# codeandkey/kami

Measured on AMD Instinct MI355X. Metric: NN leaf-evals/sec at batch 512 (119×8×8 planes), 1/2/4/8 MI355X, higher is better.
Workload: dtype bf16

## Files before the change

kami_amd/csrc/kh_api.hip:

```cpp
#include "kh_internal.h"
#include "torch_archive.h"
#include "torch_archive_write.h"

#include <sched.h>
#include <atomic>
#include <chrono>
#include <thread>
#include <cmath>
#include <condition_variable>
#include <cstdarg>
#include <cstdio>
#include <cstdlib>
#include <cstring>
#include <memory>
#include <mutex>
#include <random>
#include <algorithm>
#include <string>
#include <vector>

namespace {

thread_local std::string g_err;

// ... 117 lines not shown
    uint32_t u;
    memcpy(&u, &f, 4);
    if ((u & 0x7fffffffu) > 0x7f800000u) return (uint16_t)((u >> 16) | 0x40);
    u += 0x7fffu + ((u >> 16) & 1u);
    return (uint16_t)(u >> 16);
}
uint16_t f2f16(float f)
{
    _Float16 h = (_Float16)f;
    uint16_t r;
    memcpy(&r, &h, 2);
    return r;
}

void pack_layer(std::vector<uint16_t>& out, int dtype, const float* w, const float* scale, int Co, int Ci,
                int taps, int KS, int MS, int ci0 = 0, bool centre_first = false, int perm = 0, bool pad = true)
{
    int kstep = 0;
    for (int ti = 0; ti < taps; ++ti) {
        const int tap = !centre_first ? ti : (ti == 0 ? 4 : (ti <= 4 ? ti - 1 : ti));
        for (int ks = 0; ks < KS; ++ks, ++kstep)
            for (int ms = 0; ms < MS; ++ms)
                for (int l = 0; l < 64; ++l) {
                    const int r = l & 31, h = l >> 5;
                    for (int j = 0; j < 8; ++j) {
                        const int co = ms * 32 + r;
                        const int ci = ci0 + (kstep < perm ? 32 * (ks >> 1) + 8 * (2 * (ks & 1) + (j >> 2)) + 4 * h + (j & 3)
                                                           : ks * 16 + 8 * h + j);
                        float v = 0.0f;
                        if (co < Co && ci < Ci) v = w[((size_t)co * Ci + ci) * taps + tap] * (scale ? scale[co] : 1.0f);
                        out.push_back(dtype == KH_BF16 ? f2bf16(v) : f2f16(v));
                    }
                }
    }
    while (pad && out.size() % 4096) out.push_back(0);
// ... 154 lines not shown
    return KH_OK;
}

int build_tower(Weights& W, const HostNet& n, int dtype, int F, int C, int R)
{
    using namespace kh;
    if (C > TW_CP) { W.tw_why = "filters > 64 not supported by the MFMA tower kernel yet"; return KH_OK; }
    if (F > 128) { W.tw_why = "features > 128 not supported by the MFMA tower kernel yet"; return KH_OK; }
    const int FP = F <= 32 ? 32 : 128;
    if (tower_lds_bytes(FP, R) > 160 * 1024) { W.tw_why = "too many residual blocks for the LDS parameter area"; return KH_OK; }
    std::vector<float> sc(128), sh(128);
    std::vector<uint16_t> stream;
    std::vector<float> par((size_t)tower_par_copy_floats(R), 0.0f);
    fold_bn(n.stem, C, sc.data(), sh.data());
    if (FP == 128) {
        for (int q = 0; q < 4; ++q) pack_layer(stream, dtype, n.stem.w, sc.data(), C, F, 9, 2, 2, 32 * q, false, 0, false);
        if (stream.size() != (size_t)18 * 4096) return fail(KH_ERR_INVALID, "internal: stem stream size");
    } else {
        pack_layer(stream, dtype, n.stem.w, sc.data(), C, F, 9, FP / 16, 2);
    }
    memcpy(par.data(), sh.data(), sizeof(float) * C);
    for (int i = 0; i < 2 * R; ++i) {
        fold_bn(n.res[i], C, sc.data(), sh.data());
        pack_layer(stream, dtype, n.res[i].w, sc.data(), C, C, 9, TW_CP / 16, 2, 0, true, TW_CP / 16);
        memcpy(par.data() + (size_t)(1 + i) * TW_CP, sh.data(), sizeof(float) * C);
    }
    float* pshift1 = par.data() + (size_t)(1 + 2 * R) * TW_CP;
    fold_bn(n.pconv, KH_POLICY_MID, sc.data(), pshift1);
    pack_layer(stream, dtype, n.pconv.w, sc.data(), KH_POLICY_MID, C, 1, TW_CP / 16, 4, 0, false, TW_CP / 16);
    float* pbias2 = pshift1 + KH_POLICY_MID;
    memcpy(pbias2, n.p2b, sizeof(float) * KH_POLICY_PLANES);
    pack_layer(stream, dtype, n.p2w, nullptr, KH_POLICY_PLANES, KH_POLICY_MID, 1, KH_POLICY_MID / 16, 4, 0, false, KH_POLICY_MID / 16);
    if (((stream.size() / 4096) & 1) != 0) stream.resize(stream.size() + 4096, 0);
    float* vw = pbias2 + 128;
    float vs, vsh;
    fold_bn(n.vconv, 1, &vs, &vsh);
    for (int i = 0; i < C; ++i) vw[i] = n.vconv.w[i] * vs;
    vw[TW_CP] = vsh;
    std::vector<float> fc4((size_t)KH_VALUE_WIDTH * 64 + KH_VALUE_WIDTH);
    for (int j = 0; j < KH_VALUE_WIDTH; ++j)
        for (int k = 0; k < 64; ++k) fc4[((size_t)(k / 4) * KH_VALUE_WIDTH + j) * 4 + (k & 3)] = n.fcw[(size_t)j * 64 + k];
    memcpy(fc4.data() + (size_t)KH_VALUE_WIDTH * 64, n.fcb, sizeof(float) * KH_VALUE_WIDTH);

    W.tw_nchunks = (int)(stream.size() / 4096);
    W.tw_npar = (int)par.size();
    W.tw_FP = FP;
    int rc = 0;
// ... 1775 lines not shown
```

kami_amd/csrc/kh_internal.h:

```cpp
#pragma once
#include <hip/hip_runtime.h>
#include <stddef.h>
#include <stdint.h>

#include "../../include/kami_hip.h"

namespace kh {

void launch_encode_f32(const kh_board* d_boards, int n, float* d_planes, hipStream_t s);

void launch_gather_legal(const float* policy, const int32_t* offsets, const int32_t* actions,
                         float* priors, int B, hipStream_t s, const float* vfull = nullptr, int vstride = 0,
                         float* values = nullptr, const int* flags_in = nullptr, int* flags_out = nullptr);

void launch_signal(unsigned* host_word, unsigned serial, hipStream_t s);

struct SimpleLayer {
    const float* wt;
    const float* scale;
    const float* shift;
    int Ci, Co, taps;
    int relu;
};
void launch_simple_conv(const SimpleLayer& L, const float* in, const float* skip, float* out,
// ... 17 lines not shown
    const float* fcb;
    float* policy;
    float* vfull;
    float* logits;
    int* flags;
    const int32_t* lg_offsets = nullptr;
    const int32_t* lg_actions = nullptr;
    float* lg_priors = nullptr;
    float* lg_values = nullptr;
    int* lg_flags = nullptr;
};

__host__ __device__ constexpr int tower_par_copy_floats(int R) { return (1 + 2 * R) * TW_CP + 128 + 128 + TW_CP + 4; }
__host__ __device__ constexpr int tower_par_floats(int R) { return tower_par_copy_floats(R) + TW_NB * 64 + 16; }
int tower_lds_bytes(int FP, int R);
hipError_t launch_tower(int dtype, int FP, const TowerArgs& a, int num_cus, hipStream_t s);

struct LayersArgs {
    const float* in;
    int B, F, FP, CP, R;
    unsigned short* act_in;
    unsigned short* act[3];
    unsigned short* pmid;
    float* logits;
    float* v64;
    const unsigned short* w;
    const size_t* w_off;
    const unsigned short* w4;
    const size_t* w4_off;
    const float* shift;
// ... 35 lines not shown
```

kami_amd/csrc/tower8_mfma.hip:

```cpp
#include "tower_common.h"

#include <atomic>

namespace kh {

using f32x4_t = float __attribute__((ext_vector_type(4)));
__device__ __forceinline__ void store_wt(f32x4_t* p, f32x4_t v) { asm volatile("global_store_dwordx4 %0, %1, off sc1" ::"v"(p), "v"(v) : "memory"); }
__device__ __forceinline__ void store_wt(float* p, float v) { asm volatile("global_store_dword %0, %1, off sc1" ::"v"(p), "v"(v) : "memory"); }

constexpr int T8_LAG = 1;
struct CPipe { unsigned ring; int cslot; };

__device__ __forceinline__ unsigned cpipe_advance(CPipe& p)
{
    p.cslot = (p.cslot + 1 == RING_D) ? 0 : p.cslot + 1;
    return p.ring + p.cslot * CHUNK;
}

__device__ __forceinline__ unsigned cpipe_step(CPipe& p)
{
    asm volatile("s_barrier" ::: "memory");
    __builtin_amdgcn_sched_barrier(0);
    p.cslot = (p.cslot + 1 == RING_D) ? 0 : p.cslot + 1;
    return p.ring + p.cslot * CHUNK;
// ... 10 lines not shown
                 "global_load_lds_dwordx4 %1, %2 offset:2048\n\tglobal_load_lds_dwordx4 %1, %2 offset:3072\n\t"
                 "s_mov_b32 m0, %0"
                 : "=&s"(keep) : "v"(voff), "s"(sbase), "s"(dst) : "memory");
    p.next = (p.next + 1 == p.nch) ? 0 : p.next + 1;
    p.islot = (p.islot + 1 == RING_D) ? 0 : p.islot + 1;
}

template <int VMX>
__device__ __forceinline__ void hpipe_step(Pipe& p, int hw, int lane)
{
    asm volatile("s_waitcnt vmcnt(%0)" ::"n"(4 * (RING_D - 3 - T8_LAG) + VMX) : "memory");
    asm volatile("s_barrier" ::: "memory");
    pipe_issue4(p, hw, lane);
}

template <typename T, int TAPS, int KS, int MS, int PAR, int NREG = 0, bool CF = false, int TAILV = 0>
__device__ __forceinline__ void gemm8_layer(CPipe& p, const char* smem, int lane, unsigned b_base, int stride,
                                            f32x16 (&acc)[MS], typename Elem<T>::vec8 (&A)[2][8],
                                            const typename Elem<T>::vec8* breg = nullptr)
{
    using V = typename Elem<T>::vec8;
    using S = LayerShape<TAPS, KS, MS>;
    constexpr int KPC = S::KPC;
    V B[2][KPC];
#pragma unroll
    for (int k = 0; k < KPC; ++k) {
        if (k < NREG) B[PAR][k] = breg[k];
        else B[PAR][k] = *reinterpret_cast<const V*>(smem + b_base + b_offset<TAPS, KS, CF>(k, stride));
    }
#pragma unroll
    for (int n = 0; n < S::NCH; ++n) {
        const int cur = (PAR + n) & 1, nxt = cur ^ 1;
        const unsigned a_off = cpipe_step(p) + lane * 16;
#pragma unroll
        for (int f = 0; f < 8; ++f) A[nxt][f] = *reinterpret_cast<const V*>(smem + a_off + f * 1024);
        if (n + 1 < S::NCH) {
#pragma unroll
            for (int k = 0; k < KPC; ++k) {
                if ((n + 1) * KPC + k < NREG) B[nxt][k] = breg[(n + 1) * KPC + k];
                else B[nxt][k] = *reinterpret_cast<const V*>(smem + b_base + b_offset<TAPS, KS, CF>((n + 1) * KPC + k, stride));
            }
        }
        if (TAILV > 0 && n == S::NCH - 1) {
#pragma unroll
            for (int ms = 0; ms < MS; ++ms)
#pragma unroll
                for (int k = 0; k < KPC; ++k) acc[ms] = Elem<T>::mfma(A[cur][k * MS + ms], B[cur][k], acc[ms]);
#pragma unroll
            for (int i = 0; i < KPC; ++i) {
                __builtin_amdgcn_sched_group_barrier(0x100, 2, 0);
                __builtin_amdgcn_sched_group_barrier(0x008, 1, 0);
            }
#pragma unroll
            for (int i = 0; i < (MS - 1) * KPC; ++i) {
                __builtin_amdgcn_sched_group_barrier(0x008, 1, 0);
// ... 11 lines not shown
            __builtin_amdgcn_sched_group_barrier(0x008, 1, 0);
        }
    }
}

template <typename T, int PAR>
__device__ __forceinline__ void gemm8_dummy(CPipe& p, const char* smem, int lane, typename Elem<T>::vec8 (&A)[2][8])
{
    using V = typename Elem<T>::vec8;
    const unsigned a_off = cpipe_step(p) + lane * 16;
#pragma unroll
    for (int f = 0; f < 8; ++f) A[PAR ^ 1][f] = *reinterpret_cast<const V*>(smem + a_off + f * 1024);
}


enum { BM_RASTER = 0, BM_CENTRE = 1, BM_QUARTERS = 2 };
template <int TAPS, int KS, int BM>
__device__ __forceinline__ constexpr unsigned b_off8(int kk, int stride)
{
    if constexpr (BM == BM_QUARTERS) {
        const int pass = kk / (TAPS * KS / 4), k = kk % (TAPS * KS / 4);
        return b_offset<TAPS, KS / 4, false>(k, stride) + pass * (KS / 4) * 32;
    }
    return b_offset<TAPS, KS, BM == BM_CENTRE>(kk, stride);
}

template <typename T, int TAPS, int KS, int MS, int PAR, int NREG, int BM, int N0, int N1, bool BARMID = false>
__device__ __forceinline__ void gemm8_steps(CPipe& p, const char* smem, int lane, unsigned b_base, int stride,
                                            f32x16 (&acc)[MS], typename Elem<T>::vec8 (&A)[2][8],
                                            typename Elem<T>::vec8 (&B)[2][8 / MS],
                                            const typename Elem<T>::vec8* breg = nullptr)
{
    using V = typename Elem<T>::vec8;
    using S = LayerShape<TAPS, KS, MS>;
    constexpr int KPC = S::KPC;
#pragma unroll
    for (int n = N0; n < N1; ++n) {
        const int cur = (PAR + n) & 1, nxt = cur ^ 1;
        if (BARMID && n == N0) {
            static_assert(!BARMID || (MS == 2 && KPC == 4), "mid-step barrier: 2 x 4 chunk");
            const unsigned a_off = cpipe_advance(p) + lane * 16;
#pragma unroll
            for (int k = 0; k < 2; ++k) {
#pragma unroll
                for (int ms = 0; ms < 2; ++ms) {
                    const int i = 2 * k + ms;
                    A[nxt][2 * i] = *reinterpret_cast<const V*>(smem + a_off + (2 * i) * 1024);
                    A[nxt][2 * i + 1] = *reinterpret_cast<const V*>(smem + a_off + (2 * i + 1) * 1024);
                    acc[ms] = Elem<T>::mfma(A[cur][k * MS + ms], B[cur][k], acc[ms]);
                    __builtin_amdgcn_sched_barrier(0);
                }
            }
            asm volatile("s_barrier" ::: "memory");
#pragma unroll
            for (int k = 2; k < 4; ++k) {
#pragma unroll
                for (int ms = 0; ms < 2; ++ms) {
                    if (k == 2 && n + 1 < S::NCH) {
#pragma unroll
                        for (int j = 0; j < 2; ++j) {
                            const int kk = 2 * ms + j;
                            if ((n + 1) * KPC + kk < NREG) B[nxt][kk] = breg[(n + 1) * KPC + kk];
                            else B[nxt][kk] = *reinterpret_cast<const V*>(smem + b_base + b_off8<TAPS, KS, BM>((n + 1) * KPC + kk, stride));
                        }
                    }
                    acc[ms] = Elem<T>::mfma(A[cur][k * MS + ms], B[cur][k], acc[ms]);
                    __builtin_amdgcn_sched_barrier(0);
                }
            }
            continue;
        }
        const unsigned a_off = cpipe_step(p) + lane * 16;
#pragma unroll
        for (int f = 0; f < 8; ++f) A[nxt][f] = *reinterpret_cast<const V*>(smem + a_off + f * 1024);
        if (n + 1 < S::NCH) {
#pragma unroll
            for (int k = 0; k < KPC; ++k) {
                if ((n + 1) * KPC + k < NREG) B[nxt][k] = breg[(n + 1) * KPC + k];
                else B[nxt][k] = *reinterpret_cast<const V*>(smem + b_base + b_off8<TAPS, KS, BM>((n + 1) * KPC + k, stride));
            }
        }
#pragma unroll
        for (int k = 0; k < KPC; ++k)
#pragma unroll
            for (int ms = 0; ms < MS; ++ms) acc[ms] = Elem<T>::mfma(A[cur][k * MS + ms], B[cur][k], acc[ms]);
#pragma unroll
        for (int i = 0; i < 8; ++i) {
            __builtin_amdgcn_sched_group_barrier(0x100, 2, 0);
            __builtin_amdgcn_sched_group_barrier(0x008, 1, 0);
        }
    }
}

enum { EPI_STEM = 0, EPI_PACK = 1, EPI_RESID = 2 };

template <typename T, int EPI, int G>
__device__ __forceinline__ u32x2 epi_group(const f32x16& acc, f32x16& xf)
{
    u32x2 o;
    if (EPI == EPI_PACK) {
        o.x = relu_pk(pack2<T>(acc[4 * G + 0], acc[4 * G + 1]));
        o.y = relu_pk(pack2<T>(acc[4 * G + 2], acc[4 * G + 3]));
    } else {
// ... 1 lines not shown
        for (int i = 0; i < 4; ++i) {
            const float t = relu_nan(acc[4 * G + i]);
            xf[4 * G + i] = EPI == EPI_RESID ? xf[4 * G + i] + t : t;
        }
        o.x = pack2<T>(xf[4 * G + 0], xf[4 * G + 1]);
        o.y = pack2<T>(xf[4 * G + 2], xf[4 * G + 3]);
    }
    return o;
}

#define T8_FENCE() __builtin_amdgcn_sched_barrier(0)

template <typename T, int EPI, int CURP>
__device__ __forceinline__ void boundary(CPipe& p, char* smem, int lane, f32x16 (&acc)[2], f32x16 (&nacc)[2],
                                         unsigned nshift, typename Elem<T>::vec8 (&A)[2][8],
                                         typename Elem<T>::vec8 (&B)[2][4], f32x16 (&xf)[2], unsigned out_pix, unsigned nb_base)
{
    using V = typename Elem<T>::vec8;
    constexpr int cur = CURP, nxt = CURP ^ 1;
    u32x2 o[2][4];
#define T8_LDN(ms, g) do { const float4 s_ = *reinterpret_cast<const float4*>(smem + nshift + ((ms) * 32 + 8 * (g)) * 4); \
        nacc[ms][4 * (g) + 0] = s_.x; nacc[ms][4 * (g) + 1] = s_.y; nacc[ms][4 * (g) + 2] = s_.z; nacc[ms][4 * (g) + 3] = s_.w; } while (0)
#define T8_ST(t, g) (*reinterpret_cast<u32x2*>(smem + out_pix + ((t) * 32 + 8 * (g)) * 2) = o[t][g])
#define T8_FRAG(ks) __builtin_bit_cast(V, (u32x4){ o[(ks) >> 1][2 * ((ks) & 1)].x, o[(ks) >> 1][2 * ((ks) & 1)].y, \
                                                   o[(ks) >> 1][2 * ((ks) & 1) + 1].x, o[(ks) >> 1][2 * ((ks) & 1) + 1].y })
    const unsigned a_off = cpipe_step(p) + lane * 16;
#define T8_RDA(set, f, off) (A[set][f] = *reinterpret_cast<const V*>(smem + (off) + (f) * 1024))
    T8_LDN(0, 0); T8_LDN(0, 1); acc[0] = Elem<T>::mfma(A[cur][0], B[cur][0], acc[0]); T8_FENCE();
    T8_LDN(0, 2); T8_LDN(0, 3); acc[0] = Elem<T>::mfma(A[cur][2], B[cur][1], acc[0]); T8_FENCE();
    T8_LDN(1, 0); T8_LDN(1, 1); acc[0] = Elem<T>::mfma(A[cur][4], B[cur][2], acc[0]); T8_FENCE();
    T8_LDN(1, 2); T8_LDN(1, 3); acc[0] = Elem<T>::mfma(A[cur][6], B[cur][3], acc[0]); T8_FENCE();
    T8_RDA(nxt, 0, a_off); T8_RDA(nxt, 1, a_off); acc[1] = Elem<T>::mfma(A[cur][1], B[cur][0], acc[1]); T8_FENCE();
    T8_RDA(nxt, 2, a_off); T8_RDA(nxt, 3, a_off); acc[1] = Elem<T>::mfma(A[cur][3], B[cur][1], acc[1]); T8_FENCE();
    T8_RDA(nxt, 4, a_off); T8_RDA(nxt, 5, a_off);
    o[0][0] = epi_group<T, EPI, 0>(acc[0], xf[0]); o[0][1] = epi_group<T, EPI, 1>(acc[0], xf[0]);
    acc[1] = Elem<T>::mfma(A[cur][5], B[cur][2], acc[1]); T8_FENCE();
    T8_RDA(nxt, 6, a_off); T8_RDA(nxt, 7, a_off);
    o[0][2] = epi_group<T, EPI, 2>(acc[0], xf[0]); o[0][3] = epi_group<T, EPI, 3>(acc[0], xf[0]);
    acc[1] = Elem<T>::mfma(A[cur][7], B[cur][3], acc[1]); T8_FENCE();
    const unsigned a2 = cpipe_advance(p) + lane * 16;
    {
        const V f0 = T8_FRAG(0);
        T8_ST(0, 0); T8_ST(0, 1); T8_RDA(cur, 0, a2);
        nacc[0] = Elem<T>::mfma(A[nxt][0], f0, nacc[0]); T8_FENCE();
        T8_ST(0, 2); T8_ST(0, 3); T8_RDA(cur, 1, a2);
        nacc[1] = Elem<T>::mfma(A[nxt][1], f0, nacc[1]); T8_FENCE();
    }
    {
        const V f1 = T8_FRAG(1);
        T8_RDA(cur, 2, a2); T8_RDA(cur, 3, a2);
        nacc[0] = Elem<T>::mfma(A[nxt][2], f1, nacc[0]); T8_FENCE();
        T8_RDA(cur, 4, a2); T8_RDA(cur, 5, a2);
        o[1][0] = epi_group<T, EPI, 0>(acc[1], xf[1]); o[1][1] = epi_group<T, EPI, 1>(acc[1], xf[1]);
        nacc[1] = Elem<T>::mfma(A[nxt][3], f1, nacc[1]); T8_FENCE();
    }
    {
        const V f2 = T8_FRAG(2);
        o[1][2] = epi_group<T, EPI, 2>(acc[1], xf[1]); o[1][3] = epi_group<T, EPI, 3>(acc[1], xf[1]);
        T8_ST(1, 0); T8_ST(1, 1); T8_ST(1, 2); T8_ST(1, 3);
        nacc[0] = Elem<T>::mfma(A[nxt][4], f2, nacc[0]); T8_FENCE();
        T8_RDA(cur, 6, a2); T8_RDA(cur, 7, a2);
        nacc[1] = Elem<T>::mfma(A[nxt][5], f2, nacc[1]); T8_FENCE();
    }
    {
        const V f3 = T8_FRAG(3);
        asm volatile("s_waitcnt lgkmcnt(2)\n\ts_barrier" ::: "memory");
#pragma unroll
        for (int k = 0; k < 4; ++k) B[cur][k] = *reinterpret_cast<const V*>(smem + nb_base + b_offset<9, TW_CP / 16, true>(4 + k, XSTR));
        nacc[0] = Elem<T>::mfma(A[nxt][6], f3, nacc[0]); T8_FENCE();
        nacc[1] = Elem<T>::mfma(A[nxt][7], f3, nacc[1]); T8_FENCE();
    }
#undef T8_LDN
#undef T8_ST
}

template <typename T, int EPI, int CURP>
__device__ __forceinline__ void tower_tail(CPipe& p, const char* smem, int lane, f32x16 (&acc)[2], typename Elem<T>::vec8 (&A)[2][8],
                                           typename Elem<T>::vec8 (&B)[2][4], f32x16 (&xf)[2], Packed<2>& xk)
{
    using V = typename Elem<T>::vec8;
    constexpr int cur = CURP, nxt = CURP ^ 1;
    const unsigned a_off = cpipe_step(p) + lane * 16;
    T8_RDA(nxt, 0, a_off); T8_RDA(nxt, 1, a_off); acc[0] = Elem<T>::mfma(A[cur][0], B[cur][0], acc[0]); T8_FENCE();
    T8_RDA(nxt, 2, a_off); T8_RDA(nxt, 3, a_off); acc[0] = Elem<T>::mfma(A[cur][2], B[cur][1], acc[0]); T8_FENCE();
    T8_RDA(nxt, 4, a_off); T8_RDA(nxt, 5, a_off); acc[0] = Elem<T>::mfma(A[cur][4], B[cur][2], acc[0]); T8_FENCE();
    T8_RDA(nxt, 6, a_off); T8_RDA(nxt, 7, a_off); acc[0] = Elem<T>::mfma(A[cur][6], B[cur][3], acc[0]); T8_FENCE();
    acc[1] = Elem<T>::mfma(A[cur][1], B[cur][0], acc[1]); T8_FENCE();
    acc[1] = Elem<T>::mfma(A[cur][3], B[cur][1], acc[1]); T8_FENCE();
    xk.o[0][0] = epi_group<T, EPI, 0>(acc[0], xf[0]); xk.o[0][1] = epi_group<T, EPI, 1>(acc[0], xf[0]);
    acc[1] = Elem<T>::mfma(A[cur][5], B[cur][2], acc[1]); T8_FENCE();
    xk.o[0][2] = epi_group<T, EPI, 2>(acc[0], xf[0]); xk.o[0][3] = epi_group<T, EPI, 3>(acc[0], xf[0]);
    acc[1] = Elem<T>::mfma(A[cur][7], B[cur][3], acc[1]); T8_FENCE();
    xk.o[1][0] = epi_group<T, EPI, 0>(acc[1], xf[1]); xk.o[1][1] = epi_group<T, EPI, 1>(acc[1], xf[1]);
    xk.o[1][2] = epi_group<T, EPI, 2>(acc[1], xf[1]); xk.o[1][3] = epi_group<T, EPI, 3>(acc[1], xf[1]);
}
#undef T8_RDA

template <int STRIDE>
__device__ __forceinline__ void zero_halo(char* base, int board_bytes, int t)
{
    const u32x4 z = { 0, 0, 0, 0 };
    for (int i = t; i < TW_NB * NPIX; i += 256) {
        const int pp = i % NPIX, yy = pp / PITCH, xx = pp % PITCH;
        if (yy >= 1 && yy <= 8 && xx >= 1 && xx <= 8) continue;
        char* d = base + (i / NPIX) * board_bytes + pp * STRIDE;
#pragma unroll
        for (int k = 0; k < STRIDE / 16; ++k) *reinterpret_cast<u32x4*>(d + k * 16) = z;
    }
}

template <bool LEGAL>
__device__ __forceinline__ void helper_value_fc(const TowerArgs& a, const float* v64, int b0, int j, int lane)
{
    asm volatile("s_barrier" ::: "memory");
    unsigned voff = (unsigned)j * 16u;
    asm volatile("" : "+v"(voff));
    float4 fcw[16];
#pragma unroll
    for (int k = 0; k < 16; ++k)
        fcw[k] = *reinterpret_cast<const float4*>(reinterpret_cast<const char*>(a.fcw4) + (size_t)k * KH_VALUE_WIDTH * 16 + voff);
    const float fcbias = a.fcb[j];
    __builtin_amdgcn_sched_barrier(0);
// ... 64 lines not shown
    if (wave >= 6) {
        const int pt = tid & 127;
        for (int grp = blockIdx.x; grp < ngroups; grp += gridDim.x) {
            const int b0 = grp * TW_NB;
            if (KS_STEM == 8) {
                float4_u pl[4][8];
                const int lc = pt & 7;
                const int nb = min(TW_NB, a.B - b0);
                const char* gbase = reinterpret_cast<const char*>(a.in + (size_t)b0 * 64 * F);
                unsigned voff[8];
#pragma unroll
                for (int j = 0; j < 8; ++j) {
                    const int ip = (pt >> 3) + 16 * j;
                    voff[j] = (unsigned)((min(ip >> 6, nb - 1) * 64 + (ip & 63)) * F) * 4u;
                }
                const unsigned sdst = LDS_ST + ((((pt >> 6) + 1) * PITCH + ((pt >> 3) & 7) + 1) * SSTR) + 8 * lc;
                unsigned badmax = 0u;
                auto request = [&](int q) {
                    const unsigned cc = (unsigned)min(32 * q + 4 * lc, F - 4) * 4u;
#pragma unroll
                    for (int j = 0; j < 8; ++j)
                        pl[q][j] = __builtin_nontemporal_load(reinterpret_cast<const float4_u*>(gbase + voff[j] + cc));
                };
                auto convert = [&](int q, int j) {
                    float x[4] = { pl[q][j].x, pl[q][j].y, pl[q][j].z, pl[q][j].w };
                    if (32 * q + 32 > F) {
                        const int c = 32 * q + 4 * lc;
                        const int sh = c - min(c, F - 4);
                        float y[4];
#pragma unroll
                        for (int k = 0; k < 4; ++k) {
// ... 26 lines not shown
                }
                const bool bad = badmax >= 0x7f800000u;
                if (__any(bad) && lane == 0) raise_flag<LEGAL>(a, 0);
            } else {
                if (a.boards) {
                    const int bb = pt >> 6, p = pt & 63;
                    float v[32];
#pragma unroll
                    for (int k = 0; k < 32; ++k) v[k] = 0.0f;
                    if (b0 + bb < a.B) {
                        float w[KH_NFEATURES];
                        encode_square(a.boards + (b0 + bb), p, w);
#pragma unroll
                        for (int k = 0; k < KH_NFEATURES; ++k) v[k] = w[k];
                    }
                    char* dst = smem + LDS_ST + bb * SBOARD + (((p >> 3) + 1) * PITCH + (p & 7) + 1) * SSTR;
#pragma unroll
                    for (int c = 0; c < 4; ++c) {
                        u32x4 o;
                        o.x = pack2<T>(v[8 * c + 0], v[8 * c + 1]); o.y = pack2<T>(v[8 * c + 2], v[8 * c + 3]);
                        o.z = pack2<T>(v[8 * c + 4], v[8 * c + 5]); o.w = pack2<T>(v[8 * c + 6], v[8 * c + 7]);
                        *reinterpret_cast<u32x4*>(dst + c * 16) = o;
                    }
                } else {
                    constexpr int CH = FP / 8;
                    constexpr int NIT = TW_NB * 64 * CH / 128;
                    float vin[NIT][8];
                    const int c0 = (pt % CH) * 8;
#pragma unroll
                    for (int j = 0; j < NIT; ++j) {
                        const int i = pt + 128 * j;
// ... 12 lines not shown
                    }
                    bool bad = false;
#pragma unroll
                    for (int j = 0; j < NIT; ++j) {
                        const int i = pt + 128 * j;
                        const int bb = i / (64 * CH), p = (i / CH) & 63;
                        u32x4 o;
                        unsigned w[4];
#pragma unroll
                        for (int k = 0; k < 4; ++k) {
                            const float lo = vin[j][2 * k], hi = vin[j][2 * k + 1];
                            bad = bad || !__builtin_isfinite(lo) || !__builtin_isfinite(hi);
                            w[k] = pack2<T>(lo, hi);
                        }
                        o.x = w[0]; o.y = w[1]; o.z = w[2]; o.w = w[3];
                        *reinterpret_cast<u32x4*>(smem + LDS_ST + bb * SBOARD + (((p >> 3) + 1) * PITCH + (p & 7) + 1) * SSTR + (pt % CH) * 16) = o;
                    }
                    if (__any(bad) && lane == 0) raise_flag<LEGAL>(a, 0);
                }
                lds_barrier();
                for (int i = 0; i < NSTEM; ++i) asm volatile("s_barrier" ::: "memory");
            }
            const int nsteps = 2 * R * NLAYER + NPOL;
            for (int i = 0; i < nsteps; ++i) {
                asm volatile("s_barrier" ::: "memory");
                if (i == 0 && R > 0) {
                    for (int z = 0; z < 2; ++z) zero_halo<XSTR>(smem + LDS_ST, XBOARD, pt + 128 * z);
                    asm volatile("s_waitcnt lgkmcnt(0)" ::: "memory");
                }
            }
            helper_value_fc<LEGAL>(a, v64, b0, tid & 255, lane);
// ... 5 lines not shown
        Pipe pipe;
        pipe.stream = a.wstream; pipe.nch = a.nchunks; pipe.next = 0; pipe.islot = 0; pipe.ring = LDS_RING;
#pragma unroll
        for (int i = 0; i < RING_D - 1; ++i) pipe_issue4(pipe, hw, lane);

        for (int grp = blockIdx.x; grp < ngroups; grp += gridDim.x) {
            asm volatile("s_waitcnt vmcnt(%0)\n\ts_barrier" ::"n"(4 * (RING_D - 3)) : "memory");
            for (int i = 0; i < nsteps; ++i) hpipe_step<0>(pipe, hw, lane);
            helper_value_fc<LEGAL>(a, v64, grp * TW_NB, tid & 255, lane);
            asm volatile("s_barrier" ::: "memory");
        }
        asm volatile("s_waitcnt vmcnt(0)" ::: "memory");
    } else {
        const int h = lane >> 5;
        const int wb = cw >> 1;
        const int lp = PIXMAP[lane & 31];
        const int py = 4 * (cw & 1) + (lp >> 3), px = lp & 7;
        const unsigned xin = LDS_X + wb * XBOARD + (py * PITCH + px) * XSTR + h * 16;
        const unsigned tin = LDS_ST + wb * XBOARD + (py * PITCH + px) * XSTR + h * 16;
        const unsigned sin = LDS_ST + wb * SBOARD + (py * PITCH + px) * SSTR + h * 16;
        const unsigned xout = LDS_X + wb * XBOARD + ((py + 1) * PITCH + px + 1) * XSTR;
        const unsigned tout = LDS_ST + wb * XBOARD + ((py + 1) * PITCH + px + 1) * XSTR;
        unsigned xout_h = xout + 8 * h, tout_h = tout + 8 * h, sh0 = LDS_PAR + 16 * h;
        asm volatile("" : "+v"(xout_h), "+v"(tout_h), "+v"(sh0));

        CPipe pipe;
        pipe.ring = LDS_RING; pipe.cslot = 0;
        {
            const float4* src = reinterpret_cast<const float4*>(a.params);
            float4* dst = reinterpret_cast<float4*>(par);
            const int n4 = a.npar >> 2;
            for (int i0 = 0; i0 < n4; i0 += 4 * 256) {
                const float4 v0 = src[min(i0 + ct, n4 - 1)], v1 = src[min(i0 + 256 + ct, n4 - 1)];
                const float4 v2 = src[min(i0 + 512 + ct, n4 - 1)], v3 = src[min(i0 + 768 + ct, n4 - 1)];
                if (i0 + ct < n4) dst[i0 + ct] = v0;
                if (i0 + 256 + ct < n4) dst[i0 + 256 + ct] = v1;
                if (i0 + 512 + ct < n4) dst[i0 + 512 + ct] = v2;
// ... 9 lines not shown
            zero_halo<XSTR>(smem + LDS_X, XBOARD, ct);
            zero_halo<SSTR>(smem + LDS_ST, SBOARD, ct);
            lds_barrier();
            if (first) {
                first = false;
#pragma unroll
                for (int f = 0; f < 8; ++f) A[0][f] = *reinterpret_cast<const V*>(smem + LDS_RING + lane * 16 + f * 1024);
            }

            Packed<2> xk;
            f32x16 xf[2];
#pragma unroll
            for (int i = 0; i < 16; ++i) { xf[0][i] = 0.0f; xf[1][i] = 0.0f; }
            f32x16 accA[2], accB[2];
            V B[2][4];
            acc_init<2>(accA, shift3, h);
            {
                constexpr int BMS = KS_STEM == 8 ? BM_QUARTERS : BM_RASTER;
#pragma unroll
                for (int k = 0; k < 4; ++k) B[0][k] = *reinterpret_cast<const V*>(smem + sin + b_off8<9, KS_STEM, BMS>(k, SSTR));
                gemm8_steps<T, 9, KS_STEM, 2, 0, 0, BMS, 0, NSTEM - 1>(pipe, smem, lane, sin, SSTR, accA, A, B);
            }
            constexpr int CP1 = P1 ^ 1;
            for (int r = 0; r < R; ++r) {
                boundary<T, EPI_RESID, CP1>(pipe, smem, lane, accA, accB, sh0 + (1 + 2 * r) * TW_CP * 4, A, B, xf, xout_h, xin);
                gemm8_steps<T, 9, TW_CP / 16, 2, P1, 4, BM_CENTRE, 1, 8, true>(pipe, smem, lane, xin, XSTR, accB, A, B);
                boundary<T, EPI_PACK, P1>(pipe, smem, lane, accB, accA, sh0 + (2 + 2 * r) * TW_CP * 4, A, B, xf, tout_h, tin);
                gemm8_steps<T, 9, TW_CP / 16, 2, P1 ^ 1, 4, BM_CENTRE, 1, 8, true>(pipe, smem, lane, tin, XSTR, accA, A, B);
            }
            tower_tail<T, EPI_RESID, CP1>(pipe, smem, lane, accA, A, B, xf, xk);

            {
                f32x2 s01 = { 0.0f, 0.0f }, s23 = { 0.0f, 0.0f };
#pragma unroll
                for (int ms = 0; ms < 2; ++ms)
#pragma unroll
                    for (int g = 0; g < 4; ++g) {
                        using f32x4 = float __attribute__((ext_vector_type(4)));
                        const f32x4 w = *reinterpret_cast<const f32x4*>(vw + ms * 32 + 8 * g + 4 * h);
                        const f32x2 x01 = { xf[ms][4 * g + 0], xf[ms][4 * g + 1] }, x23 = { xf[ms][4 * g + 2], xf[ms][4 * g + 3] };
                        s01 = x01 * w.xy + s01;
                        s23 = x23 * w.zw + s23;
                    }
// ... 140 lines not shown
```

kami_amd/csrc/tower_common.h:

```cpp
#pragma once
#include "kh_internal.h"
#include "encode_square.h"

namespace kh {

using bf16x8 = __attribute__((ext_vector_type(8))) __bf16;
using f16x8 = __attribute__((ext_vector_type(8))) _Float16;
using f32x16 = __attribute__((ext_vector_type(16))) float;
using u32x4 = __attribute__((ext_vector_type(4))) unsigned;
using u32x2 = __attribute__((ext_vector_type(2))) unsigned;
using float4_u = float __attribute__((ext_vector_type(4), aligned(4)));

constexpr int PITCH = 12;
constexpr int NPIX = 10 * PITCH;
constexpr int XSTR = TW_CP * 2 + 16;
constexpr int XBOARD = NPIX * XSTR;
constexpr int PSTR = KH_POLICY_MID * 2 + 16;
constexpr int PBOARD = 64 * PSTR;
constexpr int LBOARD = KH_PSIZE * 4;
constexpr int RING_D = 6;
constexpr int CHUNK = 8192;
constexpr int LDS_RING = 0;
constexpr int LDS_X = RING_D * CHUNK;
constexpr int LDS_ST = LDS_X + TW_NB * XBOARD;
constexpr int ST_MIN = TW_NB * LBOARD - TW_NB * XBOARD + TW_NB * PBOARD;

__host__ __device__ constexpr int st_size(int FP)
{
    int s = TW_NB * NPIX * (FP * 2 + 16);
    return s > ST_MIN ? s : ST_MIN;
}

static __device__ __constant__ const unsigned char PIXMAP[32] = {
    0, 1, 2, 3,
    8, 9, 10, 11, 12, 13, 14, 15,
    4, 5, 6, 7,
    24, 25, 26, 27,
    16, 17, 18, 19, 20, 21, 22, 23,
    28, 29, 30, 31
};

template <typename T> struct Elem;
template <> struct Elem<__bf16> {
    using vec8 = bf16x8;
    static __device__ __forceinline__ f32x16 mfma(vec8 a, vec8 b, f32x16 c) { return __builtin_amdgcn_mfma_f32_32x32x16_bf16(a, b, c, 0, 0, 0); }
};
template <> struct Elem<_Float16> {
    using vec8 = f16x8;
    static __device__ __forceinline__ f32x16 mfma(vec8 a, vec8 b, f32x16 c) { return __builtin_amdgcn_mfma_f32_32x32x16_f16(a, b, c, 0, 0, 0); }
};

using f32x2 = float __attribute__((ext_vector_type(2)));
template <typename T> __device__ __forceinline__ unsigned pack2(float lo, float hi)
{
    using T2 = T __attribute__((ext_vector_type(2)));
// ... 16 lines not shown
    int islot;
    unsigned ring;
};

__device__ __forceinline__ void lds_barrier()
{
    asm volatile("s_waitcnt lgkmcnt(0)\n\ts_barrier" ::: "memory");
}

template <int TAPS, int KS, int MS> struct LayerShape {
    static constexpr int KPC = 8 / MS;
    static constexpr int TK = TAPS * KS;
    static constexpr int NCH = (TK + KPC - 1) / KPC;
};

template <int TAPS, int KS, bool CF = false>
__device__ __forceinline__ constexpr unsigned b_offset(int kk, int stride)
{
    const int k = kk < TAPS * KS ? kk : 0;
    const int ti = k / KS, ks = k % KS;
    const int tap = !CF ? ti : (ti == 0 ? 4 : (ti <= 4 ? ti - 1 : ti));
    return (unsigned)((TAPS == 9 ? ((tap / 3) * PITCH + (tap % 3)) * stride : 0) + ks * 32);
}

template <int MS>
__device__ __forceinline__ void acc_init(f32x16 (&acc)[MS], const float* shift, int h)
{
#pragma unroll
    for (int ms = 0; ms < MS; ++ms)
#pragma unroll
        for (int g = 0; g < 4; ++g) {
            const float4 s = *reinterpret_cast<const float4*>(shift + ms * 32 + 8 * g + 4 * h);
            acc[ms][4 * g + 0] = s.x; acc[ms][4 * g + 1] = s.y; acc[ms][4 * g + 2] = s.z; acc[ms][4 * g + 3] = s.w;
        }
}

template <int MS> struct Packed { u32x2 o[MS][4]; };
// ... 56 lines not shown
```

Baseline: 16.10 million.

## Derive horizontal 3x3 conv taps via DPP lane shifts instead of LDS reads

The 3x3 tower convolutions now load only the dx=0 column of each tap row from LDS. The dx=-1 and dx=+1 fragments are built from it with DPP row shifts (0x111/0x101), and lanes at the board edges are masked to zero. Because columns no longer need halo padding, the LDS board pitch drops from 12 to 8 and the pixel permutation table is removed. Weights are reordered to match the new tap order. This cuts LDS read traffic and footprint, at the cost of extra VALU DPP work and tighter scheduling constraints, with correctness depending on the lane-to-pixel mapping matching DPP row-shift semantics.

```diff
diff --git a/kami_amd/csrc/kh_api.hip b/kami_amd/csrc/kh_api.hip
--- a/kami_amd/csrc/kh_api.hip
+++ b/kami_amd/csrc/kh_api.hip
@@ -155,11 +155,11 @@
 }
 
 void pack_layer(std::vector<uint16_t>& out, int dtype, const float* w, const float* scale, int Co, int Ci,
-                int taps, int KS, int MS, int ci0 = 0, bool centre_first = false, int perm = 0, bool pad = true)
+                int taps, int KS, int MS, int ci0 = 0, int perm = 0, bool pad = true)
 {
     int kstep = 0;
     for (int ti = 0; ti < taps; ++ti) {
-        const int tap = !centre_first ? ti : (ti == 0 ? 4 : (ti <= 4 ? ti - 1 : ti));
+        const int tap = taps == 9 ? kh::tower_tap(ti) : ti;
         for (int ks = 0; ks < KS; ++ks, ++kstep)
             for (int ms = 0; ms < MS; ++ms)
                 for (int l = 0; l < 64; ++l) {
@@ -344,7 +344,7 @@
     std::vector<float> par((size_t)tower_par_copy_floats(R), 0.0f);
     fold_bn(n.stem, C, sc.data(), sh.data());
     if (FP == 128) {
-        for (int q = 0; q < 4; ++q) pack_layer(stream, dtype, n.stem.w, sc.data(), C, F, 9, 2, 2, 32 * q, false, 0, false);
+        for (int q = 0; q < 4; ++q) pack_layer(stream, dtype, n.stem.w, sc.data(), C, F, 9, 2, 2, 32 * q, 0, false);
         if (stream.size() != (size_t)18 * 4096) return fail(KH_ERR_INVALID, "internal: stem stream size");
     } else {
         pack_layer(stream, dtype, n.stem.w, sc.data(), C, F, 9, FP / 16, 2);
@@ -352,15 +352,15 @@
     memcpy(par.data(), sh.data(), sizeof(float) * C);
     for (int i = 0; i < 2 * R; ++i) {
         fold_bn(n.res[i], C, sc.data(), sh.data());
-        pack_layer(stream, dtype, n.res[i].w, sc.data(), C, C, 9, TW_CP / 16, 2, 0, true, TW_CP / 16);
+        pack_layer(stream, dtype, n.res[i].w, sc.data(), C, C, 9, TW_CP / 16, 2, 0, 3 * TW_CP / 16);
         memcpy(par.data() + (size_t)(1 + i) * TW_CP, sh.data(), sizeof(float) * C);
     }
     float* pshift1 = par.data() + (size_t)(1 + 2 * R) * TW_CP;
     fold_bn(n.pconv, KH_POLICY_MID, sc.data(), pshift1);
-    pack_layer(stream, dtype, n.pconv.w, sc.data(), KH_POLICY_MID, C, 1, TW_CP / 16, 4, 0, false, TW_CP / 16);
+    pack_layer(stream, dtype, n.pconv.w, sc.data(), KH_POLICY_MID, C, 1, TW_CP / 16, 4, 0, TW_CP / 16);
     float* pbias2 = pshift1 + KH_POLICY_MID;
     memcpy(pbias2, n.p2b, sizeof(float) * KH_POLICY_PLANES);
-    pack_layer(stream, dtype, n.p2w, nullptr, KH_POLICY_PLANES, KH_POLICY_MID, 1, KH_POLICY_MID / 16, 4, 0, false, KH_POLICY_MID / 16);
+    pack_layer(stream, dtype, n.p2w, nullptr, KH_POLICY_PLANES, KH_POLICY_MID, 1, KH_POLICY_MID / 16, 4, 0, KH_POLICY_MID / 16);
     if (((stream.size() / 4096) & 1) != 0) stream.resize(stream.size() + 4096, 0);
     float* vw = pbias2 + 128;
     float vs, vsh;
diff --git a/kami_amd/csrc/kh_internal.h b/kami_amd/csrc/kh_internal.h
--- a/kami_amd/csrc/kh_internal.h
+++ b/kami_amd/csrc/kh_internal.h
@@ -55,6 +55,11 @@
 __host__ __device__ constexpr int tower_par_copy_floats(int R) { return (1 + 2 * R) * TW_CP + 128 + 128 + TW_CP + 4; }
 __host__ __device__ constexpr int tower_par_floats(int R) { return tower_par_copy_floats(R) + TW_NB * 64 + 16; }
 int tower_lds_bytes(int FP, int R);
+__host__ __device__ constexpr int tower_tap(int ti)
+{
+    const int dy = ti / 3 == 0 ? 0 : (ti / 3 == 1 ? -1 : 1), dx = ti % 3 == 0 ? 0 : (ti % 3 == 1 ? -1 : 1);
+    return (dy + 1) * 3 + dx + 1;
+}
 hipError_t launch_tower(int dtype, int FP, const TowerArgs& a, int num_cus, hipStream_t s);
 
 struct LayersArgs {
diff --git a/kami_amd/csrc/tower8_mfma.hip b/kami_amd/csrc/tower8_mfma.hip
--- a/kami_amd/csrc/tower8_mfma.hip
+++ b/kami_amd/csrc/tower8_mfma.hip
@@ -48,11 +48,12 @@
     pipe_issue4(p, hw, lane);
 }
 
-template <typename T, int TAPS, int KS, int MS, int PAR, int NREG = 0, bool CF = false, int TAILV = 0>
+template <typename T, int TAPS, int KS, int MS, int PAR, int NREG = 0, int TAILV = 0>
 __device__ __forceinline__ void gemm8_layer(CPipe& p, const char* smem, int lane, unsigned b_base, int stride,
                                             f32x16 (&acc)[MS], typename Elem<T>::vec8 (&A)[2][8],
                                             const typename Elem<T>::vec8* breg = nullptr)
 {
+    static_assert(TAPS == 1, "3x3 layers run through gemm8_steps / boundary");
     using V = typename Elem<T>::vec8;
     using S = LayerShape<TAPS, KS, MS>;
     constexpr int KPC = S::KPC;
@@ -60,7 +61,7 @@
 #pragma unroll
     for (int k = 0; k < KPC; ++k) {
         if (k < NREG) B[PAR][k] = breg[k];
-        else B[PAR][k] = *reinterpret_cast<const V*>(smem + b_base + b_offset<TAPS, KS, CF>(k, stride));
+        else B[PAR][k] = *reinterpret_cast<const V*>(smem + b_base + b_offset1<KS>(k));
     }
 #pragma unroll
     for (int n = 0; n < S::NCH; ++n) {
@@ -72,7 +73,7 @@
 #pragma unroll
             for (int k = 0; k < KPC; ++k) {
                 if ((n + 1) * KPC + k < NREG) B[nxt][k] = breg[(n + 1) * KPC + k];
-                else B[nxt][k] = *reinterpret_cast<const V*>(smem + b_base + b_offset<TAPS, KS, CF>((n + 1) * KPC + k, stride));
+                else B[nxt][k] = *reinterpret_cast<const V*>(smem + b_base + b_offset1<KS>((n + 1) * KPC + k));
             }
         }
         if (TAILV > 0 && n == S::NCH - 1) {
@@ -114,26 +115,38 @@
 }
 
 
-enum { BM_RASTER = 0, BM_CENTRE = 1, BM_QUARTERS = 2 };
-template <int TAPS, int KS, int BM>
-__device__ __forceinline__ constexpr unsigned b_off8(int kk, int stride)
-{
-    if constexpr (BM == BM_QUARTERS) {
-        const int pass = kk / (TAPS * KS / 4), k = kk % (TAPS * KS / 4);
-        return b_offset<TAPS, KS / 4, false>(k, stride) + pass * (KS / 4) * 32;
-    }
-    return b_offset<TAPS, KS, BM == BM_CENTRE>(kk, stride);
-}
-
-template <typename T, int TAPS, int KS, int MS, int PAR, int NREG, int BM, int N0, int N1, bool BARMID = false>
+template <class W, int KPC, int PAR, typename V>
+__device__ __forceinline__ void b_fetch(int c, int k0, int k1, V (&B)[2][KPC], const char* smem, unsigned b_base, int stride,
+                                        const V* breg, unsigned ml, unsigned mr)
+{
+    const int set = (PAR + c) & 1;
+#pragma unroll
+    for (int k = k0; k < k1; ++k) {
+        const int kk = c * KPC + k, kind = W::kind(kk);
+        if (kind == BSRC_LDS) {
+            B[set][k] = *reinterpret_cast<const V*>(smem + b_base + W::off(kk, stride));
+        } else if (kind == BSRC_REG) {
+            B[set][k] = breg[kk];
+        } else if (kind == BSRC_ZERO) {
+            B[set][k] = V{};
+        } else {
+            const int sk = W::src(kk);
+            const V v = W::kind(sk) == BSRC_REG ? breg[sk] : B[(PAR + sk / KPC) & 1][sk % KPC];
+            if (kind == BSRC_SHR) B[set][k] = dpp_frag<V, 0x111>(v, ml);
+            else B[set][k] = dpp_frag<V, 0x101>(v, mr);
+        }
+    }
+}
+
+template <typename T, class W, int MS, int PAR, int N0, int N1, bool BARMID = false>
 __device__ __forceinline__ void gemm8_steps(CPipe& p, const char* smem, int lane, unsigned b_base, int stride,
                                             f32x16 (&acc)[MS], typename Elem<T>::vec8 (&A)[2][8],
                                             typename Elem<T>::vec8 (&B)[2][8 / MS],
-                                            const typename Elem<T>::vec8* breg = nullptr)
+                                            const typename Elem<T>::vec8* breg, unsigned ml, unsigned mr)
 {
     using V = typename Elem<T>::vec8;
-    using S = LayerShape<TAPS, KS, MS>;
-    constexpr int KPC = S::KPC;
+    constexpr int KPC = 8 / MS;
+    constexpr int NCH = (W::TK + KPC - 1) / KPC;
 #pragma unroll
     for (int n = N0; n < N1; ++n) {
         const int cur = (PAR + n) & 1, nxt = cur ^ 1;
@@ -156,14 +169,7 @@
             for (int k = 2; k < 4; ++k) {
 #pragma unroll
                 for (int ms = 0; ms < 2; ++ms) {
-                    if (k == 2 && n + 1 < S::NCH) {
-#pragma unroll
-                        for (int j = 0; j < 2; ++j) {
-                            const int kk = 2 * ms + j;
-                            if ((n + 1) * KPC + kk < NREG) B[nxt][kk] = breg[(n + 1) * KPC + kk];
-                            else B[nxt][kk] = *reinterpret_cast<const V*>(smem + b_base + b_off8<TAPS, KS, BM>((n + 1) * KPC + kk, stride));
-                        }
-                    }
+                    if (k == 2 && n + 1 < NCH) b_fetch<W, KPC, PAR>(n + 1, 2 * ms, 2 * ms + 2, B, smem, b_base, stride, breg, ml, mr);
                     acc[ms] = Elem<T>::mfma(A[cur][k * MS + ms], B[cur][k], acc[ms]);
                     __builtin_amdgcn_sched_barrier(0);
                 }
@@ -173,13 +179,7 @@
         const unsigned a_off = cpipe_step(p) + lane * 16;
 #pragma unroll
         for (int f = 0; f < 8; ++f) A[nxt][f] = *reinterpret_cast<const V*>(smem + a_off + f * 1024);
-        if (n + 1 < S::NCH) {
-#pragma unroll
-            for (int k = 0; k < KPC; ++k) {
-                if ((n + 1) * KPC + k < NREG) B[nxt][k] = breg[(n + 1) * KPC + k];
-                else B[nxt][k] = *reinterpret_cast<const V*>(smem + b_base + b_off8<TAPS, KS, BM>((n + 1) * KPC + k, stride));
-            }
-        }
+        if (n + 1 < NCH) b_fetch<W, KPC, PAR>(n + 1, 0, KPC, B, smem, b_base, stride, breg, ml, mr);
 #pragma unroll
         for (int k = 0; k < KPC; ++k)
 #pragma unroll
@@ -187,6 +187,7 @@
 #pragma unroll
         for (int i = 0; i < 8; ++i) {
             __builtin_amdgcn_sched_group_barrier(0x100, 2, 0);
+            __builtin_amdgcn_sched_group_barrier(0x002, 2, 0);
             __builtin_amdgcn_sched_group_barrier(0x008, 1, 0);
         }
     }
@@ -218,7 +219,8 @@
 template <typename T, int EPI, int CURP>
 __device__ __forceinline__ void boundary(CPipe& p, char* smem, int lane, f32x16 (&acc)[2], f32x16 (&nacc)[2],
                                          unsigned nshift, typename Elem<T>::vec8 (&A)[2][8],
-                                         typename Elem<T>::vec8 (&B)[2][4], f32x16 (&xf)[2], unsigned out_pix, unsigned nb_base)
+                                         typename Elem<T>::vec8 (&B)[2][4], typename Elem<T>::vec8 (&fc)[4],
+                                         f32x16 (&xf)[2], unsigned out_pix, unsigned ml)
 {
     using V = typename Elem<T>::vec8;
     constexpr int cur = CURP, nxt = CURP ^ 1;
@@ -244,35 +246,37 @@
     acc[1] = Elem<T>::mfma(A[cur][7], B[cur][3], acc[1]); T8_FENCE();
     const unsigned a2 = cpipe_advance(p) + lane * 16;
     {
-        const V f0 = T8_FRAG(0);
+        fc[0] = T8_FRAG(0);
         T8_ST(0, 0); T8_ST(0, 1); T8_RDA(cur, 0, a2);
-        nacc[0] = Elem<T>::mfma(A[nxt][0], f0, nacc[0]); T8_FENCE();
+        nacc[0] = Elem<T>::mfma(A[nxt][0], fc[0], nacc[0]); T8_FENCE();
         T8_ST(0, 2); T8_ST(0, 3); T8_RDA(cur, 1, a2);
-        nacc[1] = Elem<T>::mfma(A[nxt][1], f0, nacc[1]); T8_FENCE();
+        B[cur][0] = dpp_frag<V, 0x111>(fc[0], ml);
+        nacc[1] = Elem<T>::mfma(A[nxt][1], fc[0], nacc[1]); T8_FENCE();
     }
     {
-        const V f1 = T8_FRAG(1);
+        fc[1] = T8_FRAG(1);
         T8_RDA(cur, 2, a2); T8_RDA(cur, 3, a2);
-        nacc[0] = Elem<T>::mfma(A[nxt][2], f1, nacc[0]); T8_FENCE();
+        nacc[0] = Elem<T>::mfma(A[nxt][2], fc[1], nacc[0]); T8_FENCE();
         T8_RDA(cur, 4, a2); T8_RDA(cur, 5, a2);
         o[1][0] = epi_group<T, EPI, 0>(acc[1], xf[1]); o[1][1] = epi_group<T, EPI, 1>(acc[1], xf[1]);
-        nacc[1] = Elem<T>::mfma(A[nxt][3], f1, nacc[1]); T8_FENCE();
+        B[cur][1] = dpp_frag<V, 0x111>(fc[1], ml);
+        nacc[1] = Elem<T>::mfma(A[nxt][3], fc[1], nacc[1]); T8_FENCE();
     }
     {
-        const V f2 = T8_FRAG(2);
+        fc[2] = T8_FRAG(2);
         o[1][2] = epi_group<T, EPI, 2>(acc[1], xf[1]); o[1][3] = epi_group<T, EPI, 3>(acc[1], xf[1]);
         T8_ST(1, 0); T8_ST(1, 1); T8_ST(1, 2); T8_ST(1, 3);
-        nacc[0] = Elem<T>::mfma(A[nxt][4], f2, nacc[0]); T8_FENCE();
+        nacc[0] = Elem<T>::mfma(A[nxt][4], fc[2], nacc[0]); T8_FENCE();
         T8_RDA(cur, 6, a2); T8_RDA(cur, 7, a2);
-        nacc[1] = Elem<T>::mfma(A[nxt][5], f2, nacc[1]); T8_FENCE();
+        B[cur][2] = dpp_frag<V, 0x111>(fc[2], ml);
+        nacc[1] = Elem<T>::mfma(A[nxt][5], fc[2], nacc[1]); T8_FENCE();
     }
     {
-        const V f3 = T8_FRAG(3);
+        fc[3] = T8_FRAG(3);
         asm volatile("s_waitcnt lgkmcnt(2)\n\ts_barrier" ::: "memory");
-#pragma unroll
-        for (int k = 0; k < 4; ++k) B[cur][k] = *reinterpret_cast<const V*>(smem + nb_base + b_offset<9, TW_CP / 16, true>(4 + k, XSTR));
-        nacc[0] = Elem<T>::mfma(A[nxt][6], f3, nacc[0]); T8_FENCE();
-        nacc[1] = Elem<T>::mfma(A[nxt][7], f3, nacc[1]); T8_FENCE();
+        nacc[0] = Elem<T>::mfma(A[nxt][6], fc[3], nacc[0]); T8_FENCE();
+        B[cur][3] = dpp_frag<V, 0x111>(fc[3], ml);
+        nacc[1] = Elem<T>::mfma(A[nxt][7], fc[3], nacc[1]); T8_FENCE();
     }
 #undef T8_LDN
 #undef T8_ST
@@ -303,13 +307,12 @@
 template <int STRIDE>
 __device__ __forceinline__ void zero_halo(char* base, int board_bytes, int t)
 {
+    constexpr int NP = STRIDE / 16;
     const u32x4 z = { 0, 0, 0, 0 };
-    for (int i = t; i < TW_NB * NPIX; i += 256) {
-        const int pp = i % NPIX, yy = pp / PITCH, xx = pp % PITCH;
-        if (yy >= 1 && yy <= 8 && xx >= 1 && xx <= 8) continue;
-        char* d = base + (i / NPIX) * board_bytes + pp * STRIDE;
-#pragma unroll
-        for (int k = 0; k < STRIDE / 16; ++k) *reinterpret_cast<u32x4*>(d + k * 16) = z;
+    for (int i = t; i < TW_NB * 2 * PITCH * NP; i += 256) {
+        const int px = i / NP, hp = px % (2 * PITCH);
+        const int pp = hp < PITCH ? hp : (NPIX - 2 * PITCH) + hp;
+        *reinterpret_cast<u32x4*>(base + (px / (2 * PITCH)) * board_bytes + pp * STRIDE + (i % NP) * 16) = z;
     }
 }
 
@@ -404,7 +407,7 @@
                     const int ip = (pt >> 3) + 16 * j;
                     voff[j] = (unsigned)((min(ip >> 6, nb - 1) * 64 + (ip & 63)) * F) * 4u;
                 }
-                const unsigned sdst = LDS_ST + ((((pt >> 6) + 1) * PITCH + ((pt >> 3) & 7) + 1) * SSTR) + 8 * lc;
+                const unsigned sdst = LDS_ST + ((((pt >> 6) + 1) * PITCH + ((pt >> 3) & 7)) * SSTR) + 8 * lc;
                 unsigned badmax = 0u;
                 auto request = [&](int q) {
                     const unsigned cc = (unsigned)min(32 * q + 4 * lc, F - 4) * 4u;
@@ -461,7 +464,7 @@
 #pragma unroll
                         for (int k = 0; k < KH_NFEATURES; ++k) v[k] = w[k];
                     }
-                    char* dst = smem + LDS_ST + bb * SBOARD + (((p >> 3) + 1) * PITCH + (p & 7) + 1) * SSTR;
+                    char* dst = smem + LDS_ST + bb * SBOARD + (((p >> 3) + 1) * PITCH + (p & 7)) * SSTR;
 #pragma unroll
                     for (int c = 0; c < 4; ++c) {
                         u32x4 o;
@@ -504,7 +507,7 @@
                             w[k] = pack2<T>(lo, hi);
                         }
                         o.x = w[0]; o.y = w[1]; o.z = w[2]; o.w = w[3];
-                        *reinterpret_cast<u32x4*>(smem + LDS_ST + bb * SBOARD + (((p >> 3) + 1) * PITCH + (p & 7) + 1) * SSTR + (pt % CH) * 16) = o;
+                        *reinterpret_cast<u32x4*>(smem + LDS_ST + bb * SBOARD + (((p >> 3) + 1) * PITCH + (p & 7)) * SSTR + (pt % CH) * 16) = o;
                     }
                     if (__any(bad) && lane == 0) raise_flag<LEGAL>(a, 0);
                 }
@@ -540,13 +543,14 @@
     } else {
         const int h = lane >> 5;
         const int wb = cw >> 1;
-        const int lp = PIXMAP[lane & 31];
-        const int py = 4 * (cw & 1) + (lp >> 3), px = lp & 7;
+        const int py = 4 * (cw & 1) + ((lane & 31) >> 3), px = lane & 7;
         const unsigned xin = LDS_X + wb * XBOARD + (py * PITCH + px) * XSTR + h * 16;
         const unsigned tin = LDS_ST + wb * XBOARD + (py * PITCH + px) * XSTR + h * 16;
         const unsigned sin = LDS_ST + wb * SBOARD + (py * PITCH + px) * SSTR + h * 16;
-        const unsigned xout = LDS_X + wb * XBOARD + ((py + 1) * PITCH + px + 1) * XSTR;
-        const unsigned tout = LDS_ST + wb * XBOARD + ((py + 1) * PITCH + px + 1) * XSTR;
+        const unsigned xout = LDS_X + wb * XBOARD + ((py + 1) * PITCH + px) * XSTR;
+        const unsigned tout = LDS_ST + wb * XBOARD + ((py + 1) * PITCH + px) * XSTR;
+        unsigned ml = px != 0 ? ~0u : 0u, mr = px != 7 ? ~0u : 0u;
+        asm volatile("" : "+v"(ml), "+v"(mr));
         unsigned xout_h = xout + 8 * h, tout_h = tout + 8 * h, sh0 = LDS_PAR + 16 * h;
         asm volatile("" : "+v"(xout_h), "+v"(tout_h), "+v"(sh0));
 
@@ -586,19 +590,20 @@
             for (int i = 0; i < 16; ++i) { xf[0][i] = 0.0f; xf[1][i] = 0.0f; }
             f32x16 accA[2], accB[2];
             V B[2][4];
+            V fc[4];
             acc_init<2>(accA, shift3, h);
             {
-                constexpr int BMS = KS_STEM == 8 ? BM_QUARTERS : BM_RASTER;
-#pragma unroll
-                for (int k = 0; k < 4; ++k) B[0][k] = *reinterpret_cast<const V*>(smem + sin + b_off8<9, KS_STEM, BMS>(k, SSTR));
-                gemm8_steps<T, 9, KS_STEM, 2, 0, 0, BMS, 0, NSTEM - 1>(pipe, smem, lane, sin, SSTR, accA, A, B);
+                using WS = Win3<2, KS_STEM / 2, false>;
+                b_fetch<WS, 4, 0>(0, 0, 4, B, smem, sin, SSTR, static_cast<const V*>(nullptr), ml, mr);
+                gemm8_steps<T, WS, 2, 0, 0, NSTEM - 1>(pipe, smem, lane, sin, SSTR, accA, A, B, nullptr, ml, mr);
             }
             constexpr int CP1 = P1 ^ 1;
             for (int r = 0; r < R; ++r) {
-                boundary<T, EPI_RESID, CP1>(pipe, smem, lane, accA, accB, sh0 + (1 + 2 * r) * TW_CP * 4, A, B, xf, xout_h, xin);
-                gemm8_steps<T, 9, TW_CP / 16, 2, P1, 4, BM_CENTRE, 1, 8, true>(pipe, smem, lane, xin, XSTR, accB, A, B);
-                boundary<T, EPI_PACK, P1>(pipe, smem, lane, accB, accA, sh0 + (2 + 2 * r) * TW_CP * 4, A, B, xf, tout_h, tin);
-                gemm8_steps<T, 9, TW_CP / 16, 2, P1 ^ 1, 4, BM_CENTRE, 1, 8, true>(pipe, smem, lane, tin, XSTR, accA, A, B);
+                using WC = Win3<TW_CP / 16, 1, true>;
+                boundary<T, EPI_RESID, CP1>(pipe, smem, lane, accA, accB, sh0 + (1 + 2 * r) * TW_CP * 4, A, B, fc, xf, xout_h, ml);
+                gemm8_steps<T, WC, 2, P1, 1, 8, true>(pipe, smem, lane, xin, XSTR, accB, A, B, fc, ml, mr);
+                boundary<T, EPI_PACK, P1>(pipe, smem, lane, accB, accA, sh0 + (2 + 2 * r) * TW_CP * 4, A, B, fc, xf, tout_h, ml);
+                gemm8_steps<T, WC, 2, P1 ^ 1, 1, 8, true>(pipe, smem, lane, tin, XSTR, accA, A, B, fc, ml, mr);
             }
             tower_tail<T, EPI_RESID, CP1>(pipe, smem, lane, accA, A, B, xf, xk);
 
diff --git a/kami_amd/csrc/tower_common.h b/kami_amd/csrc/tower_common.h
--- a/kami_amd/csrc/tower_common.h
+++ b/kami_amd/csrc/tower_common.h
@@ -11,7 +11,7 @@
 using u32x2 = __attribute__((ext_vector_type(2))) unsigned;
 using float4_u = float __attribute__((ext_vector_type(4), aligned(4)));
 
-constexpr int PITCH = 12;
+constexpr int PITCH = 8;
 constexpr int NPIX = 10 * PITCH;
 constexpr int XSTR = TW_CP * 2 + 16;
 constexpr int XBOARD = NPIX * XSTR;
@@ -31,14 +31,6 @@
     return s > ST_MIN ? s : ST_MIN;
 }
 
-static __device__ __constant__ const unsigned char PIXMAP[32] = {
-    0, 1, 2, 3,
-    8, 9, 10, 11, 12, 13, 14, 15,
-    4, 5, 6, 7,
-    24, 25, 26, 27,
-    16, 17, 18, 19, 20, 21, 22, 23,
-    28, 29, 30, 31
-};
 
 template <typename T> struct Elem;
 template <> struct Elem<__bf16> {
@@ -85,13 +77,35 @@
     static constexpr int NCH = (TK + KPC - 1) / KPC;
 };
 
-template <int TAPS, int KS, bool CF = false>
-__device__ __forceinline__ constexpr unsigned b_offset(int kk, int stride)
+template <int KS>
+__device__ __forceinline__ constexpr unsigned b_offset1(int kk) { return (unsigned)((kk < KS ? kk : 0) * 32); }
+
+enum { BSRC_LDS = 0, BSRC_REG = 1, BSRC_SHR = 2, BSRC_SHL = 3, BSRC_ZERO = 4 };
+template <int KSP, int NPASS, bool REG> struct Win3 {
+    static constexpr int KP = 9 * KSP;
+    static constexpr int TK = NPASS * KP;
+    static __device__ __forceinline__ constexpr int kind(int kk)
+    {
+        if (kk >= TK) return BSRC_ZERO;
+        const int k = kk % KP, dxi = (k / KSP) % 3;
+        return dxi == 1 ? BSRC_SHR : dxi == 2 ? BSRC_SHL : (REG && k < KSP) ? BSRC_REG : BSRC_LDS;
+    }
+    static __device__ __forceinline__ constexpr int src(int kk) { return kk - ((kk % KP) / KSP) % 3 * KSP; }
+    static __device__ __forceinline__ constexpr unsigned off(int kk, int stride)
+    {
+        const int pass = kk / KP, k = kk % KP, row = k / (3 * KSP), ks = k % KSP;
+        const int dy1 = row == 0 ? 1 : (row == 1 ? 0 : 2);
+        return (unsigned)(dy1 * PITCH * stride + (pass * KSP + ks) * 32);
+    }
+};
+
+template <typename V, int CTRL>
+__device__ __forceinline__ V dpp_frag(V v, unsigned mask)
 {
-    const int k = kk < TAPS * KS ? kk : 0;
-    const int ti = k / KS, ks = k % KS;
-    const int tap = !CF ? ti : (ti == 0 ? 4 : (ti <= 4 ? ti - 1 : ti));
-    return (unsigned)((TAPS == 9 ? ((tap / 3) * PITCH + (tap % 3)) * stride : 0) + ks * 32);
+    u32x4 u = __builtin_bit_cast(u32x4, v);
+#pragma unroll
+    for (int i = 0; i < 4; ++i) u[i] = (unsigned)__builtin_amdgcn_mov_dpp((int)u[i], CTRL, 0xf, 0xf, true) & mask;
+    return __builtin_bit_cast(V, u);
 }
 
 template <int MS>
```

After: 16.00 million, median of 2. No clear change (-0.6%).
